# ralexstokes/ethereum_consensus

Hardware: NVIDIA H100
Metric: fast_aggregate_verify tuples/s (higher is better)
Workload: dtype u32 limbs (381-bit Fp), u32 SHA-256 words

## Files before the change

ethereum_consensus_b200/csrc/bls_g1.cu:

```cuda
#if defined(B200_G1_SQR_VIA_MUL)
#define B200_FP_SQR_VIA_MUL 1
#endif
#if !defined(B200_G1_INLINE_MUL)
#define B200_FP_MUL_CALL 1
#endif
#define B200_POW_TAB_SMEM 1
#include <cuda_runtime.h>

#include "../../include/b200_consensus.h"
#include "bls_kernels.cuh"

namespace b200 {
namespace {

__device__ __forceinline__ void g1_validate_body(const uint8_t* __restrict__ keys, uint32_t n, G1Aff* __restrict__ out,
                                                 int32_t* __restrict__ codes) {
    const uint32_t i = blockIdx.x * blockDim.x + threadIdx.x;
    if (i >= n) return;
    __align__(16) uint8_t b[48];
    const uint4* src = reinterpret_cast<const uint4*>(keys + size_t(i) * 48);
    uint4* dst = reinterpret_cast<uint4*>(b);
    dst[0] = src[0]; dst[1] = src[1]; dst[2] = src[2];
    G1Aff p;
    const int32_t rc = g1_key_validate(p, b);
    codes[i] = rc;
    if (rc == BLS_SUCCESS) out[i] = p;
}
__global__ void __maxnreg__(224) k_g1_validate_main(const uint8_t* __restrict__ keys, uint32_t n, G1Aff* __restrict__ out,
                                                    int32_t* __restrict__ codes) {
    g1_validate_body(keys, n, out, codes);
}
__global__ void __maxnreg__(168) k_g1_validate_r168(const uint8_t* __restrict__ keys, uint32_t n, G1Aff* __restrict__ out,
                                                    int32_t* __restrict__ codes) {
    g1_validate_body(keys, n, out, codes);
}
__global__ void __maxnreg__(128) k_g1_validate_r128(const uint8_t* __restrict__ keys, uint32_t n, G1Aff* __restrict__ out,
                                                    int32_t* __restrict__ codes) {
    g1_validate_body(keys, n, out, codes);
}
constexpr int kAggWarps = 4;

__global__ void __launch_bounds__(32 * kAggWarps) k_g1_aggregate(const G1Aff* __restrict__ keys,
                                                                  const int32_t* __restrict__ key_codes,
                                                                  const uint32_t* __restrict__ index,
                                                                  const uint32_t* __restrict__ off, uint32_t n_tuples,
                                                                  G1Aff* __restrict__ agg, G1Pre* __restrict__ agg_pre,
                                                                  int32_t* __restrict__ pk_code,
                                                                  uint32_t* __restrict__ flags, uint32_t extra_flags,
                                                                  G1Jac* __restrict__ agg_jac,
                                                                  const uint32_t* __restrict__ tuple_flags) {
    __shared__ G1Jac part[kAggWarps][32];
    const uint32_t warp = threadIdx.x >> 5, lane = threadIdx.x & 31;
    const uint32_t t = blockIdx.x * kAggWarps + warp;
    if (t >= n_tuples) return;
    const uint32_t lo = off[t], hi = off[t + 1];
    uint32_t first_bad = 0xffffffffu;
    for (uint32_t k = lo + lane; k < hi; k += 32) {
        const uint32_t id = index ? index[k] : k;
        if (key_codes[id] != BLS_SUCCESS) { first_bad = k; break; }
    }
    for (int s = 16; s > 0; s >>= 1) first_bad = min(first_bad, __shfl_xor_sync(0xffffffffu, first_bad, s));
    if (first_bad != 0xffffffffu) {
        if (lane == 0) {
            pk_code[t] = key_codes[index ? index[first_bad] : first_bad];
            flags[t] = 0;
        }
        return;
    }
    if (tuple_flags) extra_flags |= tuple_flags[t];
    if (agg == nullptr && agg_pre == nullptr) {
        if (lane == 0) { pk_code[t] = BLS_SUCCESS; flags[t] = (hi == lo ? TUPLE_FLAG_EMPTY : 0u) | extra_flags; }
        return;
    }
    G1Jac acc;
    jac_set_inf(acc);
    for (uint32_t k = lo + lane; k < hi; k += 32) {
        const G1Aff q = keys[index ? index[k] : k];
        jac_add_mixed(acc, acc, q.x, q.y);
    }
    part[warp][lane] = acc;
    __syncwarp();
    for (int s = 16; s > 0; s >>= 1) {
        if (lane < s) {
            G1Jac a = part[warp][lane], b = part[warp][lane + s];
            jac_add(a, a, b);
            part[warp][lane] = a;
        }
        __syncwarp();
    }
    if (lane == 0) {
        bool inf;
        if (agg_pre) {
            const G1Jac s = part[warp][0];
            G1Pre p;
            inf = jac_is_inf(s);
            Fp zz;
            fp_sqr(zz, s.z);
            fp_mul(p.z3, zz, s.z);
            fp_mul(p.xz, s.x, s.z);
            p.y = s.y;
            p.inf = inf ? 1u : 0u;
            agg_pre[t] = p;
            if (agg_jac) agg_jac[t] = s;
        } else {
            G1Aff a;
            jac_to_aff(a, part[warp][0]);
            agg[t] = a;
            inf = a.inf != 0;
        }
        pk_code[t] = BLS_SUCCESS;
        flags[t] = (hi == lo ? TUPLE_FLAG_EMPTY : 0u) | (inf ? TUPLE_FLAG_AGG_INF : 0u) | extra_flags;
    }
}

__global__ void k_g1_compress_groups(const G1Aff* __restrict__ agg, const int32_t* __restrict__ pk_code,
                                     const uint32_t* __restrict__ flags, uint32_t n_groups, uint8_t* __restrict__ out48,
                                     int32_t* __restrict__ out_code) {
    const uint32_t g = blockIdx.x * blockDim.x + threadIdx.x;
    if (g >= n_groups) return;
    uint8_t* o = out48 + size_t(g) * 48;
    const int32_t rc = pk_code[g] != BLS_SUCCESS ? pk_code[g] : (flags[g] & TUPLE_FLAG_EMPTY) ? int32_t(B200_EMPTY_AGGREGATE) : BLS_SUCCESS;
    out_code[g] = rc;
    if (rc == BLS_SUCCESS) g1_compress(o, agg[g]);
    else for (int k = 0; k < 48; k++) o[k] = 0;
}
__global__ void k_g1_pair_operands(const G1Aff* __restrict__ keys, const uint32_t* __restrict__ index, uint32_t n,
                                   G1Pre* __restrict__ pre, G1Aff* __restrict__ aff) {
    const uint32_t i = blockIdx.x * blockDim.x + threadIdx.x;
    if (i >= n) return;
    const G1Aff a = keys[index ? index[i] : i];
    if (pre) {
        G1Pre p;
        p.xz = a.x; p.y = a.y; p.z3 = fp_one(); p.inf = a.inf;
        pre[i] = p;
    }
    if (aff) aff[i] = a;
}
__global__ void k_neg_g1(G1Aff* out, G1Pre* out_pre) {
    if (threadIdx.x == 0 && blockIdx.x == 0) {
        G1Aff g;
        const Fp x = B200_FP_G1_X, y = B200_FP_G1_NEG_Y;
        g.x = x; g.y = y; g.inf = 0;
        *out = g;
        G1Pre p;
        p.xz = x; p.y = y; p.z3 = fp_one(); p.inf = 0;
        *out_pre = p;
    }
}

__global__ void k_fp_selftest(uint32_t n, uint32_t seed, uint32_t* out_mismatch) {
    const uint32_t i = blockIdx.x * blockDim.x + threadIdx.x;
    if (i >= n) return;
    uint64_t s = (uint64_t(seed) << 32) | i;
    auto next = [&]() { s += 0x9e3779b97f4a7c15ull; uint64_t z = s; z = (z ^ (z >> 30)) * 0xbf58476d1ce4e5b9ull;
                        z = (z ^ (z >> 27)) * 0x94d049bb133111ebull; return uint32_t((z ^ (z >> 31)) >> 16); };
    Fp a, b, c;
    for (int k = 0; k < 12; k++) { a.l[k] = next(); b.l[k] = next(); c.l[k] = next(); }
    a.l[11] &= 0x0fffffffu; b.l[11] &= 0x0fffffffu; c.l[11] &= 0x0fffffffu;
    if ((i & 7) == 1) { const Fp pp = fp_p(); Fp one; for (int k = 0; k < 12; k++) one.l[k] = 0; one.l[0] = 1 + (i >> 3); fp_sub_raw(a, pp, one); }
    Fp ab, bc, l, r, t;
    uint32_t bad = 0;
    fp_mul(ab, a, b); fp_mul(l, ab, c); fp_mul(bc, b, c); fp_mul(r, a, bc);
    if (!fp_eq(l, r)) bad++;
    fp_add(t, b, c); fp_mul(l, a, t); fp_mul(r, a, c); fp_add(r, r, ab);
    if (!fp_eq(l, r)) bad++;
    fp_sqr(l, a); fp_mul(r, a, a);
    if (!fp_eq(l, r)) bad++;
    fp_mul_portable(r, a, b);
    if (!fp_eq(ab, r)) bad++;
    fp_mul_portable(r, a, a); fp_sqr(l, a);
    if (!fp_eq(l, r)) bad++;
    {
        Fp x = a, y = b;
        if ((i & 15) == 3) y = a;
        if ((i & 15) == 5) x = fp_zero();
        if ((i & 15) == 7) { y = fp_zero(); }
        Fp u, v;
        const uint32_t cu = fp_add_raw(u, x, y), cv = fp_add_raw_portable(v, x, y);
        if (cu != cv || !fp_eq(u, v)) bad++;
        const uint32_t bu = fp_sub_raw(u, x, y), bv = fp_sub_raw_portable(v, x, y);
        if (bu != bv || !fp_eq(u, v)) bad++;
        fp_add(u, x, y); fp_sub(u, u, y);
        if (!fp_eq(u, x)) bad++;
        fp_sub(u, x, y); fp_sub(v, y, x); fp_neg(v, v);
        if (!fp_eq(u, v)) bad++;
        fp_dbl(u, x); fp_add(v, x, x);
        if (!fp_eq(u, v)) bad++;
        fp_neg(u, x); fp_add(u, u, x);
        if (!fp_is_zero(u)) bad++;
        fp_add_masked_raw(u, x, y, 0u);
        if (!fp_eq(u, x)) bad++;
        fp_add_masked_raw(u, x, y, 0xffffffffu); fp_add_raw_portable(v, x, y);
        if (!fp_eq(u, v)) bad++;
    }
    if ((i & 63) == 0 && !fp_is_zero(a)) {
        fp_inv(t, a); fp_mul(t, t, a);
        if (!fp_eq(t, fp_one())) bad++;
        Fp k, f;
        fp_inv_kaliski(k, a); fp_inv_fermat(f, a);
        if (!fp_eq(k, f)) bad++;
        fp_inv_kaliski(k, fp_zero());
        if (!fp_is_zero(k)) bad++;
    }
    if (bad) atomicAdd(out_mismatch, bad);
}

__global__ void k_fp_eval(int32_t op, uint32_t n, const uint32_t* __restrict__ a, const uint32_t* __restrict__ b,
                          uint32_t* __restrict__ out) {
    const uint32_t i = blockIdx.x * blockDim.x + threadIdx.x;
    if (i >= n) return;
    Fp x, y, x1, y1, r = fp_zero();
    for (int k = 0; k < 12; k++) { x.l[k] = a[size_t(i) * kFpEvalIn + k]; y.l[k] = b[size_t(i) * kFpEvalIn + k]; }
    for (int k = 0; k < 12; k++) { x1.l[k] = a[size_t(i) * kFpEvalIn + 12 + k]; y1.l[k] = b[size_t(i) * kFpEvalIn + 12 + k]; }
    const FpL xl = fpl_from_fp(x), yl = fpl_from_fp(y), x1l = fpl_from_fp(x1), y1l = fpl_from_fp(y1);
    FpL rl;
    uint32_t flag = 0;
    switch (op) {
    case FP_EVAL_MUL: fp_mul(r, x, y); break;
    case FP_EVAL_SQR: fp_sqr(r, x); break;
    case FPL_EVAL_MUL: f_mul(rl, xl, yl); r = rl.v; break;
    case FPL_EVAL_SQR: f_sqr(rl, xl); r = rl.v; break;
    case FP_EVAL_ADD: fp_add(r, x, y); break;
    case FP_EVAL_SUB: fp_sub(r, x, y); break;
    case FP_EVAL_NEG: fp_neg(r, x); break;
    case FPL_EVAL_ADD: f_add(rl, xl, yl); r = rl.v; break;
    case FPL_EVAL_SUB: f_sub(rl, xl, yl); r = rl.v; break;
    case FPL_EVAL_NEG: f_neg(rl, xl); r = rl.v; break;
    case FP_EVAL_ADD_RAW: flag = fp_add_raw(r, x, y); break;
    case FP_EVAL_SUB_RAW: flag = fp_sub_raw(r, x, y); break;
    case FP_EVAL_INV_KALISKI: fp_inv_kaliski(r, x); break;
    case FP_EVAL_INV_FERMAT: fp_inv_fermat(r, x); break;
    case FP_EVAL_SQRT: flag = fp_sqrt(r, x) ? 1u : 0u; break;
    case FPL_EVAL_POW_SQRT: fpl_pow(rl, xl, B200_EXP_TABLE(exp_sqrt)); r = rl.v; break;
    case FPL_EVAL_SQRT_CHAIN: fpl_sqrt_chain(rl, xl); r = rl.v; break;
    case FPL_EVAL_MUL_SUB_MUL: f_mul_sub_mul(rl, xl, x1l, yl, y1l); r = rl.v; break;
    case FPL_EVAL_MUL_SUB_8SQR: f_mul_sub_8sqr(rl, xl, x1l, yl); r = rl.v; break;
    case FP_EVAL_IS_LEX_LARGEST: flag = fp_is_lex_largest(x) ? 1u : 0u; break;
    default: break;
    }
    uint32_t* o = out + size_t(i) * kFpEvalOut;
    for (int k = 0; k < 12; k++) { o[k] = r.l[k]; o[12 + k] = 0; }
    o[24] = flag;
}

__global__ void k_curve_eval(int32_t op, uint32_t n, const uint32_t* __restrict__ a, const uint32_t* __restrict__ b,
                             uint32_t* __restrict__ out) {
    const uint32_t i = blockIdx.x * blockDim.x + threadIdx.x;
    if (i >= n) return;
    const uint32_t* pa = a + size_t(i) * kCurveEvalWords;
    const uint32_t* pb = b + size_t(i) * kCurveEvalWords;
    Jac<FpL> p, q, r;
    for (int k = 0; k < 12; k++) {
        p.x.v.l[k] = pa[k]; p.y.v.l[k] = pa[24 + k]; p.z.v.l[k] = pa[48 + k];
        q.x.v.l[k] = pb[k]; q.y.v.l[k] = pb[24 + k]; q.z.v.l[k] = pb[48 + k];
    }
    jac_set_inf(r);
    uint32_t flag = 0;
    switch (op) {
    case CURVE_G1L_ADD_MIXED: jac_add_mixed(r, p, q.x, q.y); break;
    case CURVE_G1L_ADD: jac_add(r, p, q); break;
    case CURVE_G1L_DOUBLE: jac_double(r, p); break;
    case CURVE_G1L_IN_SUBGROUP: {
        G1Aff s;
        s.x = p.x.v; s.y = p.y.v; s.inf = pa[72];
        flag = g1_in_subgroup_lazy(s) ? 1u : 0u;
        break;
    }
    default: break;
    }
    uint32_t* o = out + size_t(i) * kCurveEvalWords;
    for (int k = 0; k < 72; k++) o[k] = 0;
    for (int k = 0; k < 12; k++) { o[k] = r.x.v.l[k]; o[24 + k] = r.y.v.l[k]; o[48 + k] = r.z.v.l[k]; }
    o[72] = flag;
}

}

template <class K>
static size_t with_pow_tab(K kernel, unsigned threads) {
    const size_t bytes = fp_pow_smem_bytes(threads);
    static const void* seen[16];
    static size_t granted[16];
    static int n_seen = 0;
    const void* key = reinterpret_cast<const void*>(kernel);
    for (int i = 0; i < n_seen; i++)
        if (seen[i] == key) {
            if (granted[i] < bytes) { cudaFuncSetAttribute(kernel, cudaFuncAttributeMaxDynamicSharedMemorySize, int(bytes)); granted[i] = bytes; }
            return bytes;
        }
    cudaFuncSetAttribute(kernel, cudaFuncAttributeMaxDynamicSharedMemorySize, int(bytes));
    if (n_seen < 16) { seen[n_seen] = key; granted[n_seen++] = bytes; }
    return bytes;
}
template <class K>
static size_t k1_smem(K kernel, unsigned threads) {
#if defined(B200_G1_CANONICAL_FP)
    return with_pow_tab(kernel, threads);
#else
    (void)threads;
    static const void* done[3];
    static int n_done = 0;
    const void* key = reinterpret_cast<const void*>(kernel);
    for (int i = 0; i < n_done; i++)
        if (done[i] == key) return 0;
    cudaFuncSetAttribute(kernel, cudaFuncAttributePreferredSharedMemoryCarveout, 0);
    if (n_done < 3) done[n_done++] = key;
    return 0;
#endif
}
static int g_g1_variant = 7;
static uint32_t g_g1_small_n = 3u * 148u * 384u;
void set_g1_small_n(uint32_t n) { g_g1_small_n = n; }
void set_g1_variant(int v) { if (v >= 0 && v <= 7) g_g1_variant = v; }
void launch_g1_validate(const uint8_t* keys, uint32_t n, G1Aff* out, int32_t* codes, void* stream, int cta) {
    if (!n) return;
    cudaStream_t st = static_cast<cudaStream_t>(stream);
    switch (g_g1_variant) {
    case 6: k_g1_validate_r128<<<(n + 511) / 512, 512, k1_smem(k_g1_validate_r128, 512), st>>>(keys, n, out, codes); break;
    case 0: k_g1_validate_main<<<(n + 255) / 256, 256, k1_smem(k_g1_validate_main, 256), st>>>(keys, n, out, codes); break;
    default:
        if (cta == 128 || (cta != 384 && n <= g_g1_small_n))
            k_g1_validate_r168<<<(n + 127) / 128, 128, k1_smem(k_g1_validate_r168, 128), st>>>(keys, n, out, codes);
        else
            k_g1_validate_r168<<<(n + 383) / 384, 384, k1_smem(k_g1_validate_r168, 384), st>>>(keys, n, out, codes);
        break;
    }
}
static __global__ void k_gather_validator_keys(const uint8_t* __restrict__ records, const uint64_t* __restrict__ index, uint32_t n,
                                               uint4* __restrict__ keys) {
    const uint32_t i = blockIdx.x * blockDim.x + threadIdx.x;
    if (i >= n) return;
    const uint8_t* r = records + (index ? index[i] : uint64_t(i)) * 121;
    uint32_t w[12];
#pragma unroll
    for (int k = 0; k < 12; k++)
        w[k] = uint32_t(r[4 * k]) | uint32_t(r[4 * k + 1]) << 8 | uint32_t(r[4 * k + 2]) << 16 | uint32_t(r[4 * k + 3]) << 24;
#pragma unroll
    for (int k = 0; k < 3; k++) keys[size_t(i) * 3 + k] = make_uint4(w[4 * k], w[4 * k + 1], w[4 * k + 2], w[4 * k + 3]);
}
void launch_gather_validator_keys(const uint8_t* records, uint32_t n, uint8_t* keys, void* stream, const uint64_t* index) {
    if (!n) return;
    k_gather_validator_keys<<<(n + 255) / 256, 256, 0, static_cast<cudaStream_t>(stream)>>>(records, index, n, reinterpret_cast<uint4*>(keys));
}
void launch_g1_aggregate(const G1Aff* keys, const int32_t* key_codes, const uint32_t* index, const uint32_t* off,
                         uint32_t n_tuples, G1Aff* agg, G1Pre* agg_pre, int32_t* pk_code, uint32_t* flags,
                         uint32_t extra_flags, void* stream, G1Jac* agg_jac, const uint32_t* tuple_flags) {
    if (!n_tuples) return;
    k_g1_aggregate<<<(n_tuples + kAggWarps - 1) / kAggWarps, 32 * kAggWarps, with_pow_tab(k_g1_aggregate, 32 * kAggWarps),
                     static_cast<cudaStream_t>(stream)>>>(
        keys, key_codes, index, off, n_tuples, agg, agg_pre, pk_code, flags, extra_flags, agg_jac, tuple_flags);
}
void launch_g1_pair_operands(const G1Aff* keys, const uint32_t* index, uint32_t n, G1Pre* pre, G1Aff* aff, void* stream) {
    if (!n) return;
    k_g1_pair_operands<<<(n + 127) / 128, 128, 0, static_cast<cudaStream_t>(stream)>>>(keys, index, n, pre, aff);
}
void launch_g1_compress_groups(const G1Aff* agg, const int32_t* pk_code, const uint32_t* flags, uint32_t n_groups, uint8_t* out48,
                               int32_t* out_code, void* stream) {
    if (!n_groups) return;
    const unsigned t = n_groups <= 32 ? 32 : 128;
    k_g1_compress_groups<<<(n_groups + t - 1) / t, t, with_pow_tab(k_g1_compress_groups, t), static_cast<cudaStream_t>(stream)>>>(
        agg, pk_code, flags, n_groups, out48, out_code);
}
void launch_neg_g1(G1Aff* out, G1Pre* out_pre, void* stream) { k_neg_g1<<<1, 32, 0, static_cast<cudaStream_t>(stream)>>>(out, out_pre); }
void launch_fp_selftest(uint32_t n, uint32_t seed, uint32_t* out_mismatch, void* stream) {
    k_fp_selftest<<<(n + 127) / 128, 128, with_pow_tab(k_fp_selftest, 128), static_cast<cudaStream_t>(stream)>>>(n, seed, out_mismatch);
}
void launch_fp_eval(int32_t op, uint32_t n, const uint32_t* a, const uint32_t* b, uint32_t* out, void* stream) {
    if (!n) return;
    k_fp_eval<<<(n + 127) / 128, 128, with_pow_tab(k_fp_eval, 128), static_cast<cudaStream_t>(stream)>>>(op, n, a, b, out);
}
void launch_curve_eval(int32_t op, uint32_t n, const uint32_t* a, const uint32_t* b, uint32_t* out, void* stream) {
    if (!n) return;
    k_curve_eval<<<(n + 127) / 128, 128, with_pow_tab(k_curve_eval, 128), static_cast<cudaStream_t>(stream)>>>(op, n, a, b, out);
}

}
```

ethereum_consensus_b200/csrc/groups.cuh:

```cuda
#pragma once
#include "curve.cuh"
#include "fpl.cuh"

namespace b200 {

enum : int32_t {
    BLS_SUCCESS = 0, BLS_BAD_ENCODING = 1, BLS_POINT_NOT_ON_CURVE = 2, BLS_POINT_NOT_IN_GROUP = 3,
    BLS_AGGR_TYPE_MISMATCH = 4, BLS_VERIFY_FAIL = 5, BLS_PK_IS_INFINITY = 6, BLS_BAD_SCALAR = 7
};

typedef Aff<Fp> G1Aff;
typedef Jac<Fp> G1Jac;
typedef Aff<Fp2> G2Aff;
typedef Jac<Fp2> G2Jac;

B200_HD bool fp_from_be48_masked(Fp& r, const uint8_t* b, bool mask_flags) {
    Fp raw;
    fp_from_be_bytes_raw(raw, b);
    if (mask_flags) raw.l[11] &= 0x1fffffffu;
    const Fp p = fp_p();
    if (fp_geq_raw(raw, p)) return false;
    fp_to_mont(r, raw);
    return true;
}
B200_HD bool bytes_all_zero(const uint8_t* b, int n) {
    uint32_t acc = 0;
    for (int i = 0; i < n; i++) acc |= b[i];
    return acc == 0;
}

B200_HD int32_t g1_uncompress(G1Aff& out, const uint8_t b[48]) {
    const uint8_t f = b[0];
    out.inf = 0;
    if (!(f & 0x80)) return BLS_BAD_ENCODING;
    if (f & 0x40) {
        if ((f & 0x3f) == 0 && bytes_all_zero(b + 1, 47)) { out.inf = 1; out.x = fp_zero(); out.y = fp_zero(); return BLS_SUCCESS; }
        return BLS_BAD_ENCODING;
    }
    Fp x, y2, y;
    if (!fp_from_be48_masked(x, b, true)) return BLS_BAD_ENCODING;
    fp_sqr(y2, x);
    fp_mul(y2, y2, x);
    const Fp four = B200_FP_B_G1;
    fp_add(y2, y2, four);
    if (!fp_sqrt(y, y2)) return BLS_POINT_NOT_ON_CURVE;
    if (fp_is_lex_largest(y) != ((f & 0x20) != 0)) fp_neg(y, y);
    out.x = x; out.y = y;
    return BLS_SUCCESS;
}

B200_HD bool g1_in_subgroup(const G1Aff& p) {
    if (p.inf) return true;
    G1Jac t, t2;
    jac_mul_u64(t, p.x, p.y, B200_Z_ABS);
    jac_mul_u64_jac(t2, t, B200_Z_ABS);
    const Fp beta = B200_FP_BETA;
    Fp bx, ny;
    fp_mul(bx, p.x, beta);
    fp_neg(ny, p.y);
    return jac_eq_aff(t2, bx, ny);
}

B200_HD int32_t g1_uncompress_lazy(G1Aff& out, const uint8_t b[48]) {
    const uint8_t f = b[0];
    out.inf = 0;
    if (!(f & 0x80)) return BLS_BAD_ENCODING;
    if (f & 0x40) {
        if ((f & 0x3f) == 0 && bytes_all_zero(b + 1, 47)) { out.inf = 1; out.x = fp_zero(); out.y = fp_zero(); return BLS_SUCCESS; }
        return BLS_BAD_ENCODING;
    }
    Fp x;
    if (!fp_from_be48_masked(x, b, true)) return BLS_BAD_ENCODING;
    FpL xl = fpl_from_fp(x), y2, yl, c;
    f_sqr(y2, xl);
    f_mul(y2, y2, xl);
    f_add(y2, y2, curve_b<FpL>());
    fpl_sqrt_chain(yl, y2);
    f_sqr(c, yl);
    if (!f_eq(c, y2)) return BLS_POINT_NOT_ON_CURVE;
    Fp y = fpl_canon(yl);
    if (fp_is_lex_largest(y) != ((f & 0x20) != 0)) fp_neg(y, y);
    out.x = x; out.y = y;
    return BLS_SUCCESS;
}
B200_HD bool g1_in_subgroup_lazy(const G1Aff& p) {
    if (p.inf) return true;
    const FpL px = fpl_from_fp(p.x), py = fpl_from_fp(p.y);
    Jac<FpL> t, t2;
    jac_mul_u64(t, px, py, B200_Z_ABS);
    jac_mul_u64_jac_cached(t2, t, B200_Z_ABS);
    const Fp beta = B200_FP_BETA;
    FpL bx, ny;
    f_mul(bx, px, fpl_from_fp(beta));
    f_neg(ny, py);
    return jac_eq_aff(t2, bx, ny);
}

B200_HD int32_t g1_key_validate(G1Aff& out, const uint8_t b[48]) {
#if defined(B200_G1_CANONICAL_FP)
    int32_t rc = g1_uncompress(out, b);
    if (rc) return rc;
    if (out.inf) return BLS_PK_IS_INFINITY;
    if (!g1_in_subgroup(out)) return BLS_POINT_NOT_IN_GROUP;
#else
    int32_t rc = g1_uncompress_lazy(out, b);
    if (rc) return rc;
    if (out.inf) return BLS_PK_IS_INFINITY;
    if (!g1_in_subgroup_lazy(out)) return BLS_POINT_NOT_IN_GROUP;
#endif
    return BLS_SUCCESS;
}

B200_HD void g1_compress(uint8_t out[48], const G1Aff& a) {
    if (a.inf) { for (int i = 0; i < 48; i++) out[i] = 0; out[0] = 0xc0; return; }
    Fp raw;
    fp_from_mont(raw, a.x);
    fp_to_be_bytes_raw(out, raw);
    out[0] |= 0x80;
    if (fp_is_lex_largest(a.y)) out[0] |= 0x20;
}

B200_BIG int32_t g2_uncompress(G2Aff& out, const uint8_t b[96]) {
    const uint8_t f = b[0];
    out.inf = 0;
    if (!(f & 0x80)) return BLS_BAD_ENCODING;
    if (f & 0x40) {
        if ((f & 0x3f) == 0 && bytes_all_zero(b + 1, 95)) { out.inf = 1; out.x = fp2_zero(); out.y = fp2_zero(); return BLS_SUCCESS; }
        return BLS_BAD_ENCODING;
    }
    Fp2 x, y2, y;
    if (!fp_from_be48_masked(x.c1, b, true)) return BLS_BAD_ENCODING;
    if (!fp_from_be48_masked(x.c0, b + 48, false)) return BLS_BAD_ENCODING;
    fp2_sqr(y2, x);
    fp2_mul(y2, y2, x);
    const Fp2 bb = B200_FP2_B_G2;
    fp2_add(y2, y2, bb);
    if (!fp2_sqrt(y, y2)) return BLS_POINT_NOT_ON_CURVE;
    if (fp2_is_lex_largest(y) != ((f & 0x20) != 0)) fp2_neg(y, y);
    out.x = x; out.y = y;
    return BLS_SUCCESS;
}

B200_HD void g2_compress(uint8_t out[96], const G2Aff& a) {
    if (a.inf) { for (int i = 0; i < 96; i++) out[i] = 0; out[0] = 0xc0; return; }
    Fp raw;
    fp_from_mont(raw, a.x.c1);
    fp_to_be_bytes_raw(out, raw);
    fp_from_mont(raw, a.x.c0);
    fp_to_be_bytes_raw(out + 48, raw);
    out[0] |= 0x80;
    if (fp2_is_lex_largest(a.y)) out[0] |= 0x20;
}

B200_BIG void g2_psi(G2Jac& r, const G2Jac& p) {
    const Fp2 cx = B200_FP2_PSI_X, cy = B200_FP2_PSI_Y;
    Fp2 t;
    fp2_conj(t, p.x); fp2_mul(r.x, t, cx);
    fp2_conj(t, p.y); fp2_mul(r.y, t, cy);
    fp2_conj(r.z, p.z);
}
B200_HD void g2_psi2(G2Jac& r, const G2Jac& p) {
    const Fp c = B200_FP_PSI2_X;
    fp2_mul_fp(r.x, p.x, c);
    fp2_neg(r.y, p.y);
    r.z = p.z;
}

B200_BIG bool g2_in_subgroup(const G2Aff& q) {
    if (q.inf) return true;
    G2Jac t, qj, ps;
    jac_mul_u64(t, q.x, q.y, B200_Z_ABS);
    jac_from_aff(qj, q);
    g2_psi(ps, qj);
    Fp2 ny;
    fp2_neg(ny, ps.y);
    return jac_eq_aff(t, ps.x, ny);
}

B200_BIG void g2_clear_cofactor(G2Jac& r, const G2Jac& p) {
    G2Jac t1, t2, t3, np;
    jac_mul_u64_jac(t1, p, B200_Z_ABS);
    jac_neg(t1, t1);
    g2_psi(t2, p);
    jac_double(t3, p);
    g2_psi2(t3, t3);
    G2Jac nt2;
    jac_neg(nt2, t2);
    jac_add(t3, t3, nt2);
    jac_add(t2, t1, t2);
    jac_mul_u64_jac(t2, t2, B200_Z_ABS);
    jac_neg(t2, t2);
    jac_add(t3, t3, t2);
    jac_neg(t1, t1);
    jac_add(t3, t3, t1);
    jac_neg(np, p);
    jac_add(r, t3, np);
}

}
```

Before: 34650.

## Split G1 key validation into integer subgroup and FP64 sqrt warps

Adds a validation kernel that splits each block's threads into two roles. 256 threads run the subgroup check on an isomorphic point built from x alone, (x*u, u^2) with u = x^3+4, so they no longer wait for the square root. The other 128 threads compute the y square root with a new double-precision Montgomery arithmetic (FpD, 48-bit limbs in FMA) and pass y through shared memory. The aim is to run integer and FP64 pipes at the same time and take the long sqrt chain off the integer path. The risks are correctness of the float-based field arithmetic, the fp64 sqrt becoming the bottleneck at 128 threads per 256 keys, and the extra synchronisation.

```diff
diff --git a/ethereum_consensus_b200/csrc/bls_g1.cu b/ethereum_consensus_b200/csrc/bls_g1.cu
--- a/ethereum_consensus_b200/csrc/bls_g1.cu
+++ b/ethereum_consensus_b200/csrc/bls_g1.cu
@@ -37,6 +37,52 @@
 __global__ void __maxnreg__(128) k_g1_validate_r128(const uint8_t* __restrict__ keys, uint32_t n, G1Aff* __restrict__ out,
                                                     int32_t* __restrict__ codes) {
     g1_validate_body(keys, n, out, codes);
+}
+constexpr int kSplitIntThreads = 256, kSplitThreads = 384;
+__global__ void __maxnreg__(168) k_g1_validate_split(const uint8_t* __restrict__ keys, uint32_t n, G1Aff* __restrict__ out,
+                                                     int32_t* __restrict__ codes) {
+    __shared__ Fp s_y[kSplitIntThreads];
+    __shared__ uint8_t s_on_curve[kSplitIntThreads];
+    const uint32_t base = blockIdx.x * kSplitIntThreads;
+    __align__(16) uint8_t b[48];
+    Fp x;
+    uint32_t inf = 0;
+    bool largest = false, in_group = true;
+    int32_t rc = BLS_SUCCESS;
+    if (threadIdx.x < kSplitIntThreads) {
+        const uint32_t i = base + threadIdx.x;
+        if (i < n) {
+            const uint4* src = reinterpret_cast<const uint4*>(keys + size_t(i) * 48);
+            uint4* dst = reinterpret_cast<uint4*>(b);
+            dst[0] = src[0]; dst[1] = src[1]; dst[2] = src[2];
+            rc = g1_parse(x, inf, largest, b);
+            if (rc == BLS_SUCCESS && !inf) in_group = g1_in_subgroup_iso(x);
+        }
+    } else {
+#pragma unroll 1
+        for (uint32_t j = threadIdx.x - kSplitIntThreads; j < kSplitIntThreads; j += kSplitThreads - kSplitIntThreads) {
+            const uint32_t i = base + j;
+            if (i >= n) break;
+            const uint4* src = reinterpret_cast<const uint4*>(keys + size_t(i) * 48);
+            uint4* dst = reinterpret_cast<uint4*>(b);
+            dst[0] = src[0]; dst[1] = src[1]; dst[2] = src[2];
+            Fp y = fp_zero();
+            bool on_curve = true;
+            if (g1_parse(x, inf, largest, b) == BLS_SUCCESS && !inf) on_curve = g1_y_from_x_fpd(y, x, largest);
+            s_y[j] = y;
+            s_on_curve[j] = on_curve;
+        }
+    }
+    __syncthreads();
+    const uint32_t i = base + threadIdx.x;
+    if (threadIdx.x >= kSplitIntThreads || i >= n) return;
+    rc = g1_key_validate_code(rc, inf, s_on_curve[threadIdx.x] != 0, in_group);
+    codes[i] = rc;
+    if (rc == BLS_SUCCESS) {
+        G1Aff p;
+        p.x = x; p.y = s_y[threadIdx.x]; p.inf = 0;
+        out[i] = p;
+    }
 }
 constexpr int kAggWarps = 4;
 
@@ -298,13 +344,13 @@
     return with_pow_tab(kernel, threads);
 #else
     (void)threads;
-    static const void* done[3];
+    static const void* done[4];
     static int n_done = 0;
     const void* key = reinterpret_cast<const void*>(kernel);
     for (int i = 0; i < n_done; i++)
         if (done[i] == key) return 0;
     cudaFuncSetAttribute(kernel, cudaFuncAttributePreferredSharedMemoryCarveout, 0);
-    if (n_done < 3) done[n_done++] = key;
+    if (n_done < 4) done[n_done++] = key;
     return 0;
 #endif
 }
@@ -322,7 +368,8 @@
         if (cta == 128 || (cta != 384 && n <= g_g1_small_n))
             k_g1_validate_r168<<<(n + 127) / 128, 128, k1_smem(k_g1_validate_r168, 128), st>>>(keys, n, out, codes);
         else
-            k_g1_validate_r168<<<(n + 383) / 384, 384, k1_smem(k_g1_validate_r168, 384), st>>>(keys, n, out, codes);
+            k_g1_validate_split<<<(n + kSplitIntThreads - 1) / kSplitIntThreads, kSplitThreads,
+                                  k1_smem(k_g1_validate_split, kSplitThreads), st>>>(keys, n, out, codes);
         break;
     }
 }
diff --git a/ethereum_consensus_b200/csrc/fpd.cuh b/ethereum_consensus_b200/csrc/fpd.cuh
--- /dev/null
+++ b/ethereum_consensus_b200/csrc/fpd.cuh
@@ -0,0 +1,180 @@
+#pragma once
+#include <cmath>
+#include <cstring>
+
+#include "fpl.cuh"
+
+namespace b200 {
+
+struct FpD {
+    double l[8];
+};
+
+B200_HD double fpd_pow2(int e) {
+    const uint64_t bits = uint64_t(1023 + e) << 52;
+#if defined(__CUDA_ARCH__)
+    return __longlong_as_double(static_cast<long long>(bits));
+#else
+    double d;
+    std::memcpy(&d, &bits, sizeof d);
+    return d;
+#endif
+}
+B200_HD double fpd_k(int c) { return 1.5 * fpd_pow2(48 * c + 100); }
+B200_HD constexpr double fpd_p(int j) {
+    return j == 0 ? -21845.0
+         : j == 1 ? -86500641359361.0 * 0x1p48
+         : j == 2 ? -10839982866433.0 * 0x1p96
+         : j == 3 ? 113459389855409.0 * 0x1p144
+         : j == 4 ? 83034393350847.0 * 0x1p192
+         : j == 5 ? 73992301405303.0 * 0x1p240
+         : j == 6 ? -27924617254986.0 * 0x1p288
+         : 28591897852288.0 * 0x1p336;
+}
+constexpr double kFpdPinv = -12885098499.0;
+
+#if defined(__CUDA_ARCH__)
+B200_HD double fpd_fma(double a, double b, double c) { return __fma_rn(a, b, c); }
+#else
+B200_HD double fpd_fma(double a, double b, double c) { return std::fma(a, b, c); }
+#endif
+
+B200_HD void fpd_mac(double* t, int c, double a, double b) {
+    const double k = fpd_k(c);
+    const double hi = fpd_fma(a, b, k) - k;
+    t[c] += fpd_fma(a, b, -hi);
+    t[c + 1] += hi;
+}
+
+B200_HD void fpd_redc(FpD& r, double* t) {
+#pragma unroll
+    for (int i = 0; i < 8; i++) {
+        const double v = t[i];
+        const double h = fpd_fma(v, kFpdPinv, fpd_k(i)) - fpd_k(i);
+        const double q = fpd_fma(v, kFpdPinv, -h);
+        t[i + 1] += fpd_fma(q, fpd_p(0), v);
+#pragma unroll
+        for (int j = 1; j < 8; j++) fpd_mac(t, i + j, q, fpd_p(j));
+    }
+#pragma unroll
+    for (int c = 8; c < 15; c++) {
+        const double cy = (t[c] + fpd_k(c)) - fpd_k(c);
+        t[c] -= cy;
+        t[c + 1] += cy;
+    }
+#pragma unroll
+    for (int k = 0; k < 8; k++) r.l[k] = t[8 + k] * 0x1p-384;
+}
+
+B200_HD void fpd_mul_core(FpD& r, const FpD& a, const FpD& b) {
+    double t[16];
+#pragma unroll
+    for (int c = 0; c < 16; c++) t[c] = -0.0;
+#pragma unroll
+    for (int i = 0; i < 8; i++)
+#pragma unroll
+        for (int j = 0; j < 8; j++) fpd_mac(t, i + j, a.l[i], b.l[j]);
+    fpd_redc(r, t);
+}
+B200_HD void fpd_sqr_core(FpD& r, const FpD& a) {
+    double t[16], a2[8];
+#pragma unroll
+    for (int c = 0; c < 16; c++) t[c] = -0.0;
+#pragma unroll
+    for (int j = 1; j < 8; j++) a2[j] = a.l[j] + a.l[j];
+#pragma unroll
+    for (int i = 0; i < 8; i++) {
+        fpd_mac(t, 2 * i, a.l[i], a.l[i]);
+#pragma unroll
+        for (int j = i + 1; j < 8; j++) fpd_mac(t, i + j, a.l[i], a2[j]);
+    }
+    fpd_redc(r, t);
+}
+
+#if defined(__CUDA_ARCH__)
+static __device__ __noinline__ FpD fpd_mul_call(FpD a, FpD b) { FpD r; fpd_mul_core(r, a, b); return r; }
+static __device__ __noinline__ FpD fpd_sqr_call(FpD a) { FpD r; fpd_sqr_core(r, a); return r; }
+B200_HD void fpd_mul(FpD& r, const FpD& a, const FpD& b) { r = fpd_mul_call(a, b); }
+B200_HD void fpd_sqr(FpD& r, const FpD& a) { r = fpd_sqr_call(a); }
+#else
+B200_HD void fpd_mul(FpD& r, const FpD& a, const FpD& b) { fpd_mul_core(r, a, b); }
+B200_HD void fpd_sqr(FpD& r, const FpD& a) { fpd_sqr_core(r, a); }
+#endif
+B200_HD void fpd_sqr_n(FpD& a, int n) {
+#pragma unroll 1
+    for (int k = 0; k < n; k++) fpd_sqr(a, a);
+}
+
+B200_HD void fpd_normalize(FpD& a) {
+#pragma unroll
+    for (int k = 0; k < 7; k++) {
+        const double cy = (a.l[k] + fpd_k(k)) - fpd_k(k);
+        a.l[k] -= cy;
+        a.l[k + 1] += cy;
+    }
+}
+B200_HD void fpd_add(FpD& r, const FpD& a, const FpD& b) {
+#pragma unroll
+    for (int k = 0; k < 8; k++) r.l[k] = a.l[k] + b.l[k];
+    fpd_normalize(r);
+}
+
+B200_HD FpD fpd_from_fp(const Fp& a) {
+    FpD r;
+    int64_t carry = 0;
+#pragma unroll
+    for (int k = 0; k < 8; k++) {
+        const int w = 3 * (k >> 1);
+        const uint64_t chunk = (k & 1) ? (a.l[w + 1] >> 16) | (uint64_t(a.l[w + 2]) << 16)
+                                       : a.l[w] | (uint64_t(a.l[w + 1] & 0xffffu) << 32);
+        int64_t d = int64_t(chunk) + carry;
+        carry = 0;
+        if (k < 7 && d >= (int64_t(1) << 47)) { d -= int64_t(1) << 48; carry = 1; }
+        r.l[k] = double(d) * fpd_pow2(48 * k);
+    }
+    return r;
+}
+B200_HD FpL fpd_to_fpl(const FpD& a) {
+    FpL r;
+    int64_t carry = 0;
+#pragma unroll
+    for (int k = 0; k < 8; k++) {
+        const int64_t d = int64_t(a.l[k] * fpd_pow2(-48 * k)) + carry;
+        const uint64_t chunk = uint64_t(d) & ((uint64_t(1) << 48) - 1);
+        carry = d >> 48;
+        const int w = 3 * (k >> 1);
+        if (k & 1) {
+            r.v.l[w + 1] |= uint32_t(chunk << 16);
+            r.v.l[w + 2] = uint32_t(chunk >> 16);
+        } else {
+            r.v.l[w] = uint32_t(chunk);
+            r.v.l[w + 1] = uint32_t(chunk >> 32);
+        }
+    }
+    Fp t;
+    fp_add_masked_raw(t, r.v, fp_2p(), 0u - uint32_t(carry != 0));
+    r.v = t;
+    return r;
+}
+
+}
+
+#include "fpd_sqrt_chain.cuh"
+
+namespace b200 {
+
+B200_HD bool g1_y_from_x_fpd(Fp& y, const Fp& x, bool largest) {
+    const Fp four = B200_FP_B_G1;
+    FpD xd = fpd_from_fp(x), y2, yd, c;
+    fpd_sqr(y2, xd);
+    fpd_mul(y2, y2, xd);
+    fpd_add(y2, y2, fpd_from_fp(four));
+    fpd_sqrt_chain(yd, y2);
+    fpd_sqr(c, yd);
+    if (!fp_eq(fpl_canon(fpd_to_fpl(c)), fpl_canon(fpd_to_fpl(y2)))) return false;
+    y = fpl_canon(fpd_to_fpl(yd));
+    if (fp_is_lex_largest(y) != largest) fp_neg(y, y);
+    return true;
+}
+
+}
diff --git a/ethereum_consensus_b200/csrc/fpd_sqrt_chain.cuh b/ethereum_consensus_b200/csrc/fpd_sqrt_chain.cuh
--- /dev/null
+++ b/ethereum_consensus_b200/csrc/fpd_sqrt_chain.cuh
@@ -0,0 +1,198 @@
+#pragma once
+
+namespace b200 {
+
+B200_BIG void fpd_sqrt_chain(FpD& r, const FpD& x1) {
+    FpD x2, x3, x5, x13, x15, acc;
+    fpd_sqr(x2, x1);
+    fpd_mul(x3, x2, x1);
+    fpd_mul(x5, x3, x2);
+    x13 = x5;
+    fpd_sqr_n(x13, 1);
+    fpd_mul(x13, x13, x3);
+    fpd_mul(x15, x13, x2);
+    acc = x13;
+    fpd_sqr_n(acc, 9);
+    fpd_mul(acc, acc, x1);
+    fpd_sqr_n(acc, 4);
+    fpd_mul(acc, acc, x1);
+    fpd_sqr_n(acc, 7);
+    fpd_mul(acc, acc, x15);
+    fpd_sqr_n(acc, 4);
+    fpd_mul(acc, acc, x5);
+    fpd_sqr_n(acc, 5);
+    fpd_mul(acc, acc, x3);
+    fpd_sqr_n(acc, 1);
+    fpd_mul(acc, acc, x1);
+    fpd_sqr_n(acc, 5);
+    fpd_mul(acc, acc, x5);
+    fpd_sqr_n(acc, 4);
+    fpd_mul(acc, acc, x15);
+    fpd_sqr_n(acc, 4);
+    fpd_mul(acc, acc, x15);
+    fpd_sqr_n(acc, 1);
+    fpd_mul(acc, acc, x1);
+    fpd_sqr_n(acc, 6);
+    fpd_mul(acc, acc, x13);
+    fpd_sqr_n(acc, 6);
+    fpd_mul(acc, acc, x13);
+    fpd_sqr_n(acc, 3);
+    fpd_mul(acc, acc, x1);
+    fpd_sqr_n(acc, 5);
+    fpd_mul(acc, acc, x5);
+    fpd_sqr_n(acc, 1);
+    fpd_mul(acc, acc, x1);
+    fpd_sqr_n(acc, 7);
+    fpd_mul(acc, acc, x13);
+    fpd_sqr_n(acc, 4);
+    fpd_mul(acc, acc, x13);
+    fpd_sqr_n(acc, 6);
+    fpd_mul(acc, acc, x15);
+    fpd_sqr_n(acc, 5);
+    fpd_mul(acc, acc, x13);
+    fpd_sqr_n(acc, 1);
+    fpd_mul(acc, acc, x1);
+    fpd_sqr_n(acc, 3);
+    fpd_mul(acc, acc, x1);
+    fpd_sqr_n(acc, 8);
+    fpd_mul(acc, acc, x13);
+    fpd_sqr_n(acc, 5);
+    fpd_mul(acc, acc, x5);
+    fpd_sqr_n(acc, 4);
+    fpd_mul(acc, acc, x13);
+    fpd_sqr_n(acc, 3);
+    fpd_mul(acc, acc, x3);
+    fpd_sqr_n(acc, 6);
+    fpd_mul(acc, acc, x13);
+    fpd_sqr_n(acc, 3);
+    fpd_mul(acc, acc, x3);
+    fpd_sqr_n(acc, 3);
+    fpd_mul(acc, acc, x5);
+    fpd_sqr_n(acc, 1);
+    fpd_mul(acc, acc, x1);
+    fpd_sqr_n(acc, 3);
+    fpd_mul(acc, acc, x1);
+    fpd_sqr_n(acc, 5);
+    fpd_mul(acc, acc, x3);
+    fpd_sqr_n(acc, 3);
+    fpd_mul(acc, acc, x5);
+    fpd_sqr_n(acc, 4);
+    fpd_mul(acc, acc, x13);
+    fpd_sqr_n(acc, 5);
+    fpd_mul(acc, acc, x5);
+    fpd_sqr_n(acc, 2);
+    fpd_mul(acc, acc, x3);
+    fpd_sqr_n(acc, 5);
+    fpd_mul(acc, acc, x1);
+    fpd_sqr_n(acc, 6);
+    fpd_mul(acc, acc, x15);
+    fpd_sqr_n(acc, 4);
+    fpd_mul(acc, acc, x3);
+    fpd_sqr_n(acc, 1);
+    fpd_mul(acc, acc, x1);
+    fpd_sqr_n(acc, 7);
+    fpd_mul(acc, acc, x5);
+    fpd_sqr_n(acc, 4);
+    fpd_mul(acc, acc, x1);
+    fpd_sqr_n(acc, 5);
+    fpd_mul(acc, acc, x5);
+    fpd_sqr_n(acc, 5);
+    fpd_mul(acc, acc, x15);
+    fpd_sqr_n(acc, 4);
+    fpd_mul(acc, acc, x13);
+    fpd_sqr_n(acc, 1);
+    fpd_mul(acc, acc, x1);
+    fpd_sqr_n(acc, 4);
+    fpd_mul(acc, acc, x3);
+    fpd_sqr_n(acc, 1);
+    fpd_mul(acc, acc, x1);
+    fpd_sqr_n(acc, 4);
+    fpd_mul(acc, acc, x3);
+    fpd_sqr_n(acc, 8);
+    fpd_mul(acc, acc, x13);
+    fpd_sqr_n(acc, 5);
+    fpd_mul(acc, acc, x5);
+    fpd_sqr_n(acc, 2);
+    fpd_mul(acc, acc, x1);
+    fpd_sqr_n(acc, 9);
+    fpd_mul(acc, acc, x15);
+    fpd_sqr_n(acc, 5);
+    fpd_mul(acc, acc, x13);
+    fpd_sqr_n(acc, 3);
+    fpd_mul(acc, acc, x3);
+    fpd_sqr_n(acc, 8);
+    fpd_mul(acc, acc, x15);
+    fpd_sqr_n(acc, 3);
+    fpd_mul(acc, acc, x3);
+    fpd_sqr_n(acc, 4);
+    fpd_mul(acc, acc, x1);
+    fpd_sqr_n(acc, 3);
+    fpd_mul(acc, acc, x1);
+    fpd_sqr_n(acc, 9);
+    fpd_mul(acc, acc, x15);
+    fpd_sqr_n(acc, 4);
+    fpd_mul(acc, acc, x5);
+    fpd_sqr_n(acc, 4);
+    fpd_mul(acc, acc, x5);
+    fpd_sqr_n(acc, 4);
+    fpd_mul(acc, acc, x15);
+    fpd_sqr_n(acc, 4);
+    fpd_mul(acc, acc, x15);
+    fpd_sqr_n(acc, 4);
+    fpd_mul(acc, acc, x15);
+    fpd_sqr_n(acc, 4);
+    fpd_mul(acc, acc, x15);
+    fpd_sqr_n(acc, 4);
+    fpd_mul(acc, acc, x5);
+    fpd_sqr_n(acc, 1);
+    fpd_mul(acc, acc, x1);
+    fpd_sqr_n(acc, 6);
+    fpd_mul(acc, acc, x5);
+    fpd_sqr_n(acc, 2);
+    fpd_mul(acc, acc, x1);
+    fpd_sqr_n(acc, 6);
+    fpd_mul(acc, acc, x15);
+    fpd_sqr_n(acc, 4);
+    fpd_mul(acc, acc, x15);
+    fpd_sqr_n(acc, 4);
+    fpd_mul(acc, acc, x15);
+    fpd_sqr_n(acc, 4);
+    fpd_mul(acc, acc, x15);
+    fpd_sqr_n(acc, 2);
+    fpd_mul(acc, acc, x3);
+    fpd_sqr_n(acc, 3);
+    fpd_mul(acc, acc, x5);
+    fpd_sqr_n(acc, 2);
+    fpd_mul(acc, acc, x3);
+    fpd_sqr_n(acc, 6);
+    fpd_mul(acc, acc, x15);
+    fpd_sqr_n(acc, 4);
+    fpd_mul(acc, acc, x15);
+    fpd_sqr_n(acc, 5);
+    fpd_mul(acc, acc, x15);
+    fpd_sqr_n(acc, 4);
+    fpd_mul(acc, acc, x15);
+    fpd_sqr_n(acc, 4);
+    fpd_mul(acc, acc, x15);
+    fpd_sqr_n(acc, 4);
+    fpd_mul(acc, acc, x15);
+    fpd_sqr_n(acc, 4);
+    fpd_mul(acc, acc, x15);
+    fpd_sqr_n(acc, 4);
+    fpd_mul(acc, acc, x15);
+    fpd_sqr_n(acc, 4);
+    fpd_mul(acc, acc, x15);
+    fpd_sqr_n(acc, 4);
+    fpd_mul(acc, acc, x15);
+    fpd_sqr_n(acc, 3);
+    fpd_mul(acc, acc, x5);
+    fpd_sqr_n(acc, 4);
+    fpd_mul(acc, acc, x5);
+    fpd_sqr_n(acc, 4);
+    fpd_mul(acc, acc, x5);
+    fpd_sqr_n(acc, 3);
+    fpd_mul(acc, acc, x3);
+    r = acc;
+}
+
+}
diff --git a/ethereum_consensus_b200/csrc/groups.cuh b/ethereum_consensus_b200/csrc/groups.cuh
--- a/ethereum_consensus_b200/csrc/groups.cuh
+++ b/ethereum_consensus_b200/csrc/groups.cuh
@@ -1,6 +1,6 @@
 #pragma once
 #include "curve.cuh"
-#include "fpl.cuh"
+#include "fpd.cuh"
 
 namespace b200 {
 
@@ -94,6 +94,41 @@
     f_mul(bx, px, fpl_from_fp(beta));
     f_neg(ny, py);
     return jac_eq_aff(t2, bx, ny);
+}
+
+B200_HD int32_t g1_parse(Fp& x, uint32_t& inf, bool& largest, const uint8_t b[48]) {
+    const uint8_t f = b[0];
+    inf = 0;
+    largest = (f & 0x20) != 0;
+    if (!(f & 0x80)) return BLS_BAD_ENCODING;
+    if (f & 0x40) {
+        if ((f & 0x3f) == 0 && bytes_all_zero(b + 1, 47)) { inf = 1; return BLS_SUCCESS; }
+        return BLS_BAD_ENCODING;
+    }
+    return fp_from_be48_masked(x, b, true) ? BLS_SUCCESS : BLS_BAD_ENCODING;
+}
+B200_HD bool g1_in_subgroup_iso(const Fp& x) {
+    const FpL xl = fpl_from_fp(x);
+    FpL u, px, py;
+    f_sqr(u, xl);
+    f_mul(u, u, xl);
+    f_add(u, u, curve_b<FpL>());
+    f_mul(px, xl, u);
+    f_sqr(py, u);
+    Jac<FpL> t, t2;
+    jac_mul_u64(t, px, py, B200_Z_ABS);
+    jac_mul_u64_jac_cached(t2, t, B200_Z_ABS);
+    const Fp beta = B200_FP_BETA;
+    FpL bx, ny;
+    f_mul(bx, px, fpl_from_fp(beta));
+    f_neg(ny, py);
+    return jac_eq_aff(t2, bx, ny);
+}
+B200_HD int32_t g1_key_validate_code(int32_t parse_rc, uint32_t inf, bool on_curve, bool in_group) {
+    if (parse_rc) return parse_rc;
+    if (inf) return BLS_PK_IS_INFINITY;
+    if (!on_curve) return BLS_POINT_NOT_ON_CURVE;
+    return in_group ? BLS_SUCCESS : BLS_POINT_NOT_IN_GROUP;
 }
 
 B200_HD int32_t g1_key_validate(G1Aff& out, const uint8_t b[48]) {
```

New measurement: 37320, median of 6. 7.7% higher.
